# Plonky3/Plonky3-recursion

Hardware: AMD Instinct MI355X
Metric: prove_next_layer ms + Poseidon2 perms/s, KoalaBear 2^20-row circuit, 1/8 GPU (lower is better)
Workload: dtype u32 Montgomery (31-bit prime field, degree-4 extension); Poseidon2 hashing as exact integers in f64; 1 GPU; prove_next_layer (verifier-circuit run on the device + prove_all_tables) of the synthetic koala-bear 2^20-row recursion layer: tables const/public/alu/poseidon2/recompose, FRI blowup 4, arity<=4, 54 queries, 15-bit PoW; circuit inputs + NextLayerPrepCache resident in HBM; field=koala-bear, log_height=20, independent_proofs=1, proof_bytes=612900, parallelism=1 independent proofs, one per GPU, no data-path collective

## Files before the change

__graft_entry__.py:

```python
import os
import subprocess
import sys

ROOT = os.path.dirname(os.path.abspath(__file__))
CSRC = os.path.join(ROOT, "plonky3_recursion_amd", "csrc")
LIB = os.path.join(ROOT, "plonky3_recursion_amd", "libp3r_hip.so")
KNOBS_LIB = os.path.join(ROOT, "plonky3_recursion_amd", "knobs", "libp3r_hip.so")
HIP_SOURCES = ["p3r_core.hip", "tu_lde.hip", "tu_quotient.hip", "tu_logup.hip", "tu_mmcs4.hip", "prep_device.hip"]


def _stale(target, deps):
    if not os.path.exists(target):
        return True
    t = os.path.getmtime(target)
    return any(os.path.getmtime(d) > t for d in deps)


def _deps_of(obj):
    dep = obj + ".d"
    if not os.path.exists(dep):
        return None
    txt = open(dep).read().replace("\\\n", " ")
    return [p for p in txt.split(":", 1)[1].split() if p]


def build():
    hipcc = os.environ.get("HIPCC", "/opt/rocm/bin/hipcc")
    flags = ["-O3", "-std=c++17", "--offload-arch=gfx950", "-fPIC", "-pthread"]
    objdir = os.path.join(CSRC, ".build")
    os.makedirs(objdir, exist_ok=True)
    os.makedirs(os.path.dirname(KNOBS_LIB), exist_ok=True)
    shared = ["prep_device.hip", "tu_quotient.hip", "tu_logup.hip", "tu_mmcs4.hip"]
    knobbed = ["p3r_core.hip", "tu_lde.hip"]
    units = [(src, src + ".o", []) for src in HIP_SOURCES]
    units += [(src, src.replace(".hip", ".knobs.o"), ["-DP3R_TUNING_KNOBS"]) for src in knobbed]
    test_only = ["tu_prims_test.hip", "tu_p2f_test.hip"]
    units += [(src, src.replace(".hip", ".knobs.o"), ["-DP3R_TUNING_KNOBS"]) for src in test_only]
    pending = []
    for src, objname, extra in units:
        obj = os.path.join(objdir, objname)
        deps = _deps_of(obj)
        if deps is None or not all(os.path.exists(d) for d in deps) or _stale(obj, deps):
            pending.append((obj, [hipcc] + flags + extra + ["-MD", "-MF", obj + ".d", "-c", "-o", obj, os.path.join(CSRC, src)]))
    running, failed = [], None
    max_jobs = max(1, min(len(pending), (os.cpu_count() or 2)))
    while pending or running:
        while pending and len(running) < max_jobs:
            obj, cmd = pending.pop(0)
            running.append((obj, subprocess.Popen(cmd, cwd=CSRC)))
        obj, proc = running.pop(0)
        if proc.wait() != 0:
            for p in (obj, obj + ".d"):
                if os.path.exists(p):
                    os.remove(p)
            failed = failed or subprocess.CalledProcessError(proc.returncode, proc.args)
    if failed:
        raise failed
    for lib, objs in ((LIB, [s + ".o" for s in HIP_SOURCES]),
                      (KNOBS_LIB, [s.replace(".hip", ".knobs.o") for s in knobbed + test_only] + [s + ".o" for s in shared])):
        paths = [os.path.join(objdir, o) for o in objs]
        if _stale(lib, paths):
            subprocess.run([hipcc] + flags + ["-shared", "-o", lib] + paths, check=True, cwd=CSRC)
    subprocess.run(["make", "-C", os.path.join(ROOT, "oracle")], check=True,
                   stdout=subprocess.DEVNULL)
    subprocess.run(["make", "-C", os.path.join(ROOT, "harness")], check=True,
                   stdout=subprocess.DEVNULL, stderr=subprocess.DEVNULL)
    subprocess.run(["make", "-C", os.path.join(ROOT, "examples")], check=True, stdout=subprocess.DEVNULL)
    chk = os.path.join(ROOT, "tools", "microbench", "zk_fill_check")
    srcs = [chk + ".hip", os.path.join(CSRC, "kernels_zk.hip.h"), os.path.join(CSRC, "zk_rand.h")]
    if not os.path.exists(chk) or any(os.path.getmtime(f) > os.path.getmtime(chk) for f in srcs):
        subprocess.run([hipcc, "--offload-arch=gfx950", "-O3", "-std=c++17", "-w", "-I", CSRC, "-o", chk, chk + ".hip"], check=True)
    if ROOT not in sys.path:
        sys.path.insert(0, ROOT)
    import plonky3_recursion_amd
    from plonky3_recursion_amd import _lib
    _lib.load()


def smoke():
    if ROOT not in sys.path:
        sys.path.insert(0, ROOT)
    sys.path.insert(0, os.path.join(ROOT, "tests"))
    import numpy as np
    import oracle_lib
    import plonky3_recursion_amd as p3r

    field = "koala-bear"
    ctx = p3r.Context(field=field)
    orc = oracle_lib.Oracle()
    rng = np.random.default_rng(0)
    n = 256
    p = oracle_lib.MODULUS[field]
    inputs = rng.integers(0, p, size=(n, 16), dtype=np.uint32)
    new_start = (rng.random(n) < 0.2).astype(np.uint8)
    merkle = (rng.random(n) < 0.7).astype(np.uint8)
    bit = rng.integers(0, 2, size=n, dtype=np.uint8)
    idx = rng.integers(0, p, size=n, dtype=np.uint32)
    g = oracle_lib.GENERATOR[field]
    tr = ctx.generate_trace_rows_device(inputs, new_start, merkle, bit, idx)
    lde = ctx.coset_lde_batch_device(tr, 2, g)
    cap, tree = ctx.commit_device([lde])
    o_tr = orc.trace_rows(field, inputs, new_start, merkle, bit, idx)
    assert np.array_equal(tr.download(), o_tr), "trace fill mismatch"
    o_lde = orc.coset_lde(field, o_tr, 2, g)
    assert np.array_equal(lde.download(), o_lde), "LDE mismatch"
    ocap, otree = orc.commit(field, [o_lde], 0)
    assert np.array_equal(cap, ocap), "MMCS commitment mismatch"
    opened, proof = tree.open_batch(321)
    assert orc.verify(field, cap, [o_lde.shape], 321, opened, proof), "opening rejected by oracle"
    tree.free()
    ctx.close()
    print("smoke ok: trace fill + LDE + MMCS commit/open bit-exact vs oracle")

    import circuit_lib
    import harness_lib
    import layer_lib
    import harness_adapters as wl
    fri = dict(log_blowup=2, max_log_arity=2, cap_height=0, log_final_poly_len=2, commit_pow_bits=0,
               query_pow_bits=6, num_queries=8)
# ... 30 lines not shown
```

plonky3_recursion_amd/csrc/context.h:

```cpp
#pragma once
#include <hip/hip_runtime.h>

#include <algorithm>
#include <array>
#include <atomic>
#include <cstdarg>
#include <cstdio>
#include <cstring>
#include <exception>
#include <functional>
#include <map>
#include <memory>
#include <chrono>
#include <mutex>
#include <stdexcept>
#include <string>
#include <thread>
#include <tuple>
#include <vector>

#include "../../include/p3r.h"
#include "field.h"
#include "poseidon2.h"
#include "proof_layout.h"
// ... 356 lines not shown
};

struct DevBuf {
  uint32_t* p = nullptr;
  size_t n = 0;
  std::shared_ptr<DevPool> pool;
  DevBuf() = default;
  explicit DevBuf(size_t cells) { alloc(cells); }
  DevBuf(const DevBuf&) = delete;
  DevBuf& operator=(const DevBuf&) = delete;
  DevBuf(DevBuf&& o) noexcept : p(o.p), n(o.n), pool(std::move(o.pool)) { o.p = nullptr; o.n = 0; }
  DevBuf& operator=(DevBuf&& o) noexcept {
    if (this != &o) { release(); p = o.p; n = o.n; pool = std::move(o.pool); o.p = nullptr; o.n = 0; }
    return *this;
  }
  ~DevBuf() { release(); }
  void alloc(size_t cells) {
    release();
    if (cells) {
      pool = tls_pool();
      if (!pool) fail(P3R_EINVAL, "device allocation outside a p3r API call");
      p = static_cast<uint32_t*>(pool->get(cells * sizeof(uint32_t)));
    }
    n = cells;
  }
  void release() {
    if (p) pool->put(p, n * sizeof(uint32_t));
    p = nullptr;
    n = 0;
    pool.reset();
  }
};

inline int log2_exact(size_t x, const char* what) {
  if (x == 0 || (x & (x - 1))) fail(P3R_EINVAL, "%s (%zu) must be a power of two", what, x);
  int l = 0;
  while ((size_t(1) << l) < x) ++l;
  return l;
}

}

struct p3r_dmat {
  p3r::DevBuf buf;
  uint32_t* d = nullptr;
  size_t h = 0, w = 0;
};

struct p3r_p2_dev {
  size_t n = 0;
  std::unique_ptr<p3r_dmat> inputs;
  p3r::DevBuf flags;
  p3r::DevBuf seed;
};

struct p3r_tree {
  std::vector<const p3r_dmat*> mats;
  std::vector<std::unique_ptr<p3r_dmat>> owned;
  int salt_elems = 0;
  std::vector<std::unique_ptr<p3r_dmat>> salt_owned;
  p3r::DevBuf phase_salts;
  size_t phase_salt_stride = 0, phase_rows = 0;
  int log_max_h = 0;
  int cap_height = 0;
  size_t total_width = 0;
  std::vector<p3r::DevBuf> layers;
  int arity = 2;
  std::vector<p3r::MmcsLevel> levels;
  std::vector<size_t> layer_n;
};

namespace p3r {
struct ProfRec {
  const char* name;
  hipEvent_t a, b;
};
}

struct p3r_ctx {
  p3r_config cfg{};
  std::shared_ptr<p3r::DevPool> pool = std::make_shared<p3r::DevPool>();
  bool prof_enabled = false;
  std::vector<p3r::ProfRec> prof;
  std::vector<std::pair<std::string, double>> stage_ms;
  std::string cur_stage;
  double cur_stage_t0 = 0;
  int partial_rounds = 0;
  hipStream_t stream = nullptr;
  int n_cus = 256;
  p3r::DevBuf rc;
  p3r::DevBuf rc_f64;
  const double* rcd() const { return reinterpret_cast<const double*>(rc_f64.p); }
  size_t rcd_w32_at = 0;
  const double* rcd_w32() const { return rcd() + rcd_w32_at; }
  p3r::DevBuf p2_diag;
  std::vector<uint32_t> rc_canonical;
  std::vector<uint8_t> fri_log_arities;
  p3r::ProofLayout proof_layout;
  std::vector<uint32_t> rc_mont_host;
  std::string err;
  bool w32_diag_builtin = false;
  bool w32_unacknowledged = false;
  uint64_t zk_nonce = 0;
  uint32_t zk_key[8] = {0, 0, 0, 0, 0, 0, 0, 0};
  std::vector<uint8_t> pending_proof;
  p3r::HostStage stage;
  p3r::HostLanding landing;
  p3r::HostPost post;
  std::map<std::string, p3r::DevBuf> const_tables;

  std::map<std::pair<int, int>, p3r::DevBuf> tw_sub;
  std::map<std::pair<int, int>, std::pair<p3r::DevBuf, p3r::DevBuf>> tw4;
  std::map<std::tuple<int, int, uint32_t>, std::pair<p3r::DevBuf, p3r::DevBuf>> pre;
};

inline hipError_t fetch_small(p3r_ctx* ctx, const uint32_t* src, size_t words, uint32_t* dst) {
  if (words == 0) return hipSuccess;
  if (words <= p3r::HostPost::kWords) {
    const uint32_t* got = nullptr;
    p3r::host_mark("fetch: posted, waiting for the GPU");
    hipError_t e = ctx->post.post(ctx->stream, src, words, &got);
    p3r::host_mark("fetch: arrived");
    if (e != hipSuccess) return e;
    std::memcpy(dst, got, words * 4);
    return hipSuccess;
  }
  return p3r::copy_sync(ctx->stream, dst, src, words * 4, hipMemcpyDeviceToHost);
}
```

plonky3_recursion_amd/csrc/kernels_fri_reduce.hip.h:

```cpp
#pragma once
#include "kernels_stark.hip.h"

namespace p3r {

template <int DC>
struct FriInvJobT {
  uint32_t* inv;
  uint64_t h;
  int log_h;
  uint32_t w_h;
  uint32_t w_4;
  EW<DC> z;
  uint32_t block0;
};
using FriInvJob = FriInvJobT<4>;
template <class PP, int DC = 4>
__global__ void __launch_bounds__(kBlock)
k_fri_inv_points(const FriInvJobT<DC>* __restrict__ jobs, int n_jobs, uint32_t gen) {
  using F = Fp<PP>;
  using E = typename Chal<PP, DC>::type;
  const int j = find_job(jobs, n_jobs);
  const FriInvJobT<DC>& job = jobs[j];
  const size_t h = job.h, r0 = ((size_t)(blockIdx.x - job.block0) * kBlock + threadIdx.x) * 4;
  if (r0 >= h) return;
  const E z = e4_load<PP, DC>(job.z);
  E x[4], v[4];
  const F x0 = F::raw(gen) * F::raw(job.w_h).pow(bit_reverse((uint32_t)r0, job.log_h));
  const F x2 = x0 * F::raw(job.w_4);
  x[0] = z - E::from_base(x0);
  x[1] = z + E::from_base(x0);
  x[2] = z - E::from_base(x2);
  x[3] = z + E::from_base(x2);
  inv4<PP>(x, v);
  const gptr<uint32_t> inv = as_global(job.inv);
#pragma unroll
  for (int m = 0; m < 4; ++m)
    if (r0 + m < h)
#pragma unroll
      for (int k = 0; k < DC; ++k) inv[(size_t)k * h + r0 + m] = v[m].c[k].v;
}

struct FriVsumJob {
  const uint32_t* vals;
  uint32_t* out;
  int w;
};
template <class PP, int DC = 4>
__global__ void __launch_bounds__(kBlock)
k_fri_vsum(const FriVsumJob* __restrict__ jobs, const uint32_t* __restrict__ apow_tab ) {
  using F = Fp<PP>;
  using E = typename Chal<PP, DC>::type;
  __shared__ uint32_t sh[kBlock / 64][DC];
  const FriVsumJob job = jobs[blockIdx.x];
  const gptr<const uint32_t> vals = as_global(job.vals);
  E acc = E::zero();
  for (int c = threadIdx.x; c < job.w; c += kBlock) {
    E ap, v;
#pragma unroll
    for (int k = 0; k < DC; ++k) {
      ap.c[k] = F::raw(apow_tab[DC * c + k]);
      v.c[k] = F::raw(vals[DC * c + k]);
    }
    acc += ap * v;
  }
  const int lane = threadIdx.x & 63, wave = threadIdx.x >> 6;
#pragma unroll
  for (int k = 0; k < DC; ++k) {
    F x = acc.c[k];
#pragma unroll
    for (int off = 32; off > 0; off >>= 1) x += F::raw(__shfl_down(x.v, off));
    if (lane == 0) sh[wave][k] = x.v;
  }
  __syncthreads();
  if (threadIdx.x < DC) {
    F x = F::zero();
#pragma unroll
    for (int wv = 0; wv < kBlock / 64; ++wv) x += F::raw(sh[wv][threadIdx.x]);
    as_global(job.out)[threadIdx.x] = x.v;
  }
}

template <int DC>
struct FriReduceMatT {
  const uint32_t* mat;
  int w, n_points;
  const uint32_t* inv[2];
  const uint32_t* v[2];
  EW<DC> off[2];
};
using FriReduceMat = FriReduceMatT<4>;
struct FriReduceJob {
  uint32_t* ro;
  uint64_t h;
  uint32_t mat0, n_mats;
  uint32_t block0;
};
template <class PP, int DC = 4>
__global__ void __launch_bounds__(kBlock)
k_fri_reduce_pre(const FriReduceJob* __restrict__ jobs, int n_jobs, const FriReduceMatT<DC>* __restrict__ mats,
                 const uint32_t* __restrict__ apow_tab ) {
  using F = Fp<PP>;
  using E = typename Chal<PP, DC>::type;
  const int j = find_job(jobs, n_jobs);
  const FriReduceJob job = jobs[j];
  const size_t h = job.h, r = (size_t)(blockIdx.x - job.block0) * kBlock + threadIdx.x;
  if (r >= h) return;
  auto apow = [&](int c) {
    E ap;
#pragma unroll
    for (int k = 0; k < DC; ++k) ap.c[k] = F::raw(apow_tab[DC * c + k]);
    return ap;
  };
  E acc = E::zero();
  for (uint32_t m = 0; m < job.n_mats; ++m) {
    const FriReduceMatT<DC>& a = mats[job.mat0 + m];
    const gptr<const uint32_t> mat = as_global(a.mat);
    const int w = a.w;
    E S = E::zero(), S2 = E::zero();
    int c = 0;
    for (; c + 3 < w; c += 4) {
      const F m0 = F::raw(mat[(size_t)c * h + r]), m1 = F::raw(mat[(size_t)(c + 1) * h + r]);
      const F m2 = F::raw(mat[(size_t)(c + 2) * h + r]), m3 = F::raw(mat[(size_t)(c + 3) * h + r]);
      S += E::dot2_base(apow(c), m0, apow(c + 1), m1);
      S2 += E::dot2_base(apow(c + 2), m2, apow(c + 3), m3);
    }
    for (; c + 1 < w; c += 2)
      S += E::dot2_base(apow(c), F::raw(mat[(size_t)c * h + r]), apow(c + 1), F::raw(mat[(size_t)(c + 1) * h + r]));
    if (c < w) S += apow(c) * F::raw(mat[(size_t)c * h + r]);
    S += S2;
    for (int p = 0; p < a.n_points; ++p) {
      E inv;
#pragma unroll
      for (int k = 0; k < DC; ++k) inv.c[k] = F::raw(as_global(a.inv[p])[(size_t)k * h + r]);
      E V;
#pragma unroll
      for (int k = 0; k < DC; ++k) V.c[k] = F::raw(as_global(a.v[p])[k]);
      acc += e4_load<PP, DC>(a.off[p]) * (V - S) * inv;
    }
  }
#pragma unroll
  for (int k = 0; k < DC; ++k) as_global(job.ro)[(size_t)k * h + r] = acc.c[k].v;
}

}
```

plonky3_recursion_amd/csrc/profile.h:

```cpp
#pragma once
#include <chrono>

#include "context.h"

namespace p3r {

inline void prof_clear(p3r_ctx* ctx) {
  for (auto& r : ctx->prof) {
    (void)hipEventDestroy(r.a);
    (void)hipEventDestroy(r.b);
  }
  ctx->prof.clear();
  ctx->stage_ms.clear();
  ctx->cur_stage.clear();
}

inline void prof_stage(p3r_ctx* ctx, const char* name) {
  p3r::host_mark(name ? name : "stage end");
  if (!ctx->prof_enabled) return;
  (void)hipStreamSynchronize(ctx->stream);
  const double now = std::chrono::duration<double, std::milli>(std::chrono::steady_clock::now().time_since_epoch()).count();
  if (!ctx->cur_stage.empty()) {
    bool found = false;
    for (auto& kv : ctx->stage_ms)
      if (kv.first == ctx->cur_stage) { kv.second += now - ctx->cur_stage_t0; found = true; }
    if (!found) ctx->stage_ms.emplace_back(ctx->cur_stage, now - ctx->cur_stage_t0);
  }
  ctx->cur_stage = name ? name : "";
  ctx->cur_stage_t0 = now;
}

inline void prof_count(p3r_ctx* ctx, const char* name, double v) {
  if (!ctx->prof_enabled) return;
  const std::string key = std::string("count:") + name;
  for (auto& kv : ctx->stage_ms)
    if (kv.first == key) { kv.second += v; return; }
  ctx->stage_ms.emplace_back(key, v);
}

struct ProfScope {
  p3r_ctx* ctx;
  hipEvent_t a = nullptr, b = nullptr;
  const char* name;
  ProfScope(p3r_ctx* c, const char* n) : ctx(c), name(n) {
    if (!ctx->prof_enabled) return;
    if (hipEventCreate(&a) != hipSuccess || hipEventCreate(&b) != hipSuccess) {
      a = b = nullptr;
      return;
    }
    (void)hipEventRecord(a, ctx->stream);
  }
  ~ProfScope() {
    if (!a) return;
    (void)hipEventRecord(b, ctx->stream);
    ctx->prof.push_back(ProfRec{name, a, b});
  }
};

}
```

plonky3_recursion_amd/csrc/prove_impl.hip.h:

```cpp
#include "host_transcript.h"
#include "kernels_stark.hip.h"
#include "kernels_fri_reduce.hip.h"
#include "kernels_zk.hip.h"
#include "open_impl.hip.h"

struct p3r_prep {
  std::vector<p3r::AirParams> airs;
  std::vector<std::unique_ptr<p3r_dmat>> traces;
  std::vector<std::unique_ptr<p3r_dmat>> evals;
  std::vector<std::unique_ptr<p3r_dmat>> ldes;
  std::vector<size_t> heights;
  int zk_codewords = -1;
  const p3r_dmat* committed(size_t i) const { return evals.empty() ? traces[i].get() : evals[i].get(); }
  std::unique_ptr<p3r_tree> tree;
  std::vector<uint32_t> cap_canonical;
};

namespace {

template <class PP, int DC = 4>
EW<DC> to_e4(const typename Chal<PP, DC>::type& e) { return e4_store<PP, DC>(e); }

template <class PP, int DC = 4>
std::vector<typename Chal<PP, DC>::type> download_ef(p3r_ctx* ctx, const uint32_t* dev, size_t count) {
  std::vector<uint32_t> raw(count * DC);
  P3R_HIP(fetch_small(ctx, dev, raw.size(), raw.data()));
  std::vector<typename Chal<PP, DC>::type> out(count);
  for (size_t i = 0; i < count; ++i)
    for (int k = 0; k < DC; ++k) out[i].c[k] = Fp<PP>::raw(raw[i * DC + k]);
  return out;
}

inline ZkKey zk_key_of(const p3r_ctx* ctx, uint64_t nonce) {
  ZkKey k{};
  for (int i = 0; i < 8; ++i) k.k[i] = ctx->zk_key[i];
  k.nonce_lo = (uint32_t)nonce; k.nonce_hi = (uint32_t)(nonce >> 32);
  return k;
}

template <class PP>
void launch_zk_tiles(p3r_ctx* ctx, std::vector<ZkTileJob>& jobs, const ZkKey& key, const char* family) {
  uint64_t blocks = 0;
  for (auto& j : jobs) {
    if (2 * (uint64_t)(j.w2 | 1u) > kZkTileWords) fail(P3R_EUNSUPPORTED, "ZK fill of a matrix of %u columns", j.w2);
    j.log_tr = zk_tile_log_rows(j.rows, j.w2);
    j.block0 = (uint32_t)blocks;
    blocks += j.rows >> j.log_tr;
  }
  if (blocks >= (uint64_t(1) << 31)) fail(P3R_EUNSUPPORTED, "ZK fill launch of %llu tiles", (unsigned long long)blocks);
  if (!blocks) return;
  DevBuf d_jobs((jobs.size() * sizeof(ZkTileJob) + 3) / 4);
  P3R_HIP(ctx->stage.upload(ctx->stream, d_jobs.p, jobs.data(), jobs.size() * sizeof(ZkTileJob)));
  ProfScope ps(ctx, family);
  hipLaunchKernelGGL(k_zk_fill_tiles<PP>, dim3((unsigned)blocks), dim3(kBlock), 0, ctx->stream, reinterpret_cast<const ZkTileJob*>(d_jobs.p),
                     (int)jobs.size(), key);
  P3R_HIP(hipGetLastError());
}

template <class PP>
std::vector<std::unique_ptr<p3r_dmat>> draw_salts(p3r_ctx* ctx, const std::vector<const p3r_dmat*>& mats, int salt_round, const ZkKey& key) {
  const uint32_t S = ctx->cfg.mmcs_salt_elems;
  std::vector<std::unique_ptr<p3r_dmat>> out;
  std::vector<ZkTileJob> tj;
  for (size_t i = 0; i < mats.size(); ++i) {
    out.push_back(dmat_alloc(mats[i]->h, S));
    ZkTileJob j{};
    j.dst = out.back()->d; j.rows = mats[i]->h; j.w2 = S; j.mode = 1; j.stride = 1;
    j.stream = zk_stream_id(salt_round, i);
    tj.push_back(j);
  }
  launch_zk_tiles<PP>(ctx, tj, key, "mmcs_salts");
  return out;
}

template <class PP>
std::unique_ptr<p3r_tree> commit_dmats(p3r_ctx* ctx, const std::vector<const p3r_dmat*>& mats,
                                       std::vector<uint32_t>& cap_mont, int salt_round = -1, const ZkKey* key = nullptr) {
  auto tree = std::make_unique<p3r_tree>();
  tree->mats = mats;
  if (ctx->cfg.mmcs_salt_elems) {
    if (salt_round < 0 || !key) fail(P3R_EHIP, "internal: a commit without its salt stream under a hiding MMCS");
    tree->salt_elems = (int)ctx->cfg.mmcs_salt_elems;
    tree->salt_owned = draw_salts<PP>(ctx, mats, salt_round, *key);
    tree->mats.clear();
    for (size_t i = 0; i < mats.size(); ++i) { tree->mats.push_back(mats[i]); tree->mats.push_back(tree->salt_owned[i].get()); }
// ... 501 lines not shown
        m.z = {zeta};
        if (r == &prep_round || r == &perm_round || (r == &main_round && air_uses_next(prep->airs[m.inst])))
          m.z.push_back(zeta * F::two_adic_generator(log_n[m.inst]));
        m.job = op.open(m.ev->d, m.ev->h, (int)m.ev->w, m.shift, m.z);
      }
    auto all = op.finish();
    launch_inv_points();
    for (Round* r : rounds())
      for (Mat& m : r->mats)
        for (auto& pv : all[m.job]) {
          for (auto& v : pv) ch.observe_ext(v);
          m.vals.emplace_back(pv.begin(), pv.end() - R);
          m.codewords.emplace_back(pv.end() - R, pv.end());
        }
    check_at_zeta();
  }

  static std::array<uint64_t, 6> inv_key(int lh, const E& z) {
    std::array<uint64_t, 6> key{(uint64_t)lh, 0, 0, 0, 0, 0};
    for (int k = 0; k < DC; ++k) key[1 + k] = z.c[k].v;
    return key;
  }

  void launch_inv_points() {
    std::vector<FriInvJobT<DC>> inv_jobs;
    uint32_t inv_blocks = 0;
    for (Round* r : rounds())
      for (const Mat& m : r->mats) {
        const int lh = log_e[m.inst] + log_blowup;
        for (const E& z : m.z) {
          const auto key = inv_key(lh, z);
          if (inv_cache.count(key)) continue;
          inv_keep.emplace_back((size_t)DC << lh);
          FriInvJobT<DC> j{};
          j.inv = inv_keep.back().p;
          j.h = uint64_t(1) << lh;
          j.log_h = lh;
          if (lh < 2) fail(P3R_EINVAL, "FRI: an LDE of fewer than four rows");
          j.w_h = F::two_adic_generator(lh).v;
          j.w_4 = F::two_adic_generator(2).v;
          j.z = to_e4<PP, DC>(z);
          j.block0 = inv_blocks;
          inv_blocks += blocks_for((size_t(1) << lh) / 4);
          inv_jobs.push_back(j);
          inv_cache.emplace(key, j.inv);
        }
      }
    inv_keep.emplace_back((inv_jobs.size() * sizeof(FriInvJobT<DC>) + 3) / 4);
    P3R_HIP(ctx->stage.upload(ctx->stream, inv_keep.back().p, inv_jobs.data(), inv_jobs.size() * sizeof(FriInvJobT<DC>)));
    ProfScope ps(ctx, "fri_inv_points");
    hipLaunchKernelGGL((k_fri_inv_points<PP, DC>), dim3(inv_blocks), dim3(kBlock), 0, ctx->stream,
                       reinterpret_cast<const FriInvJobT<DC>*>(inv_keep.back().p), (int)inv_jobs.size(), gen.v);
    P3R_HIP(hipGetLastError());
  }

  void check_at_zeta() {
    E l_beta_pow[kMaxExtD + 1];
    for (int j = 0; j <= kMaxExtD; ++j) l_beta_pow[j] = e4_load<PP, DC>(lc.beta_pow[j]);
    const E l_prefix = e4_load<PP, DC>(lc.prefix);
    std::vector<std::vector<std::vector<E>>> inst_chunks(ni);
    for (const Mat& m : quot_round.mats) inst_chunks[m.inst].push_back(m.vals[0]);
    static const std::vector<E> empty;
    for (size_t i = 0; i < ni; ++i) {
      const auto& omain = main_round.mats[i].vals;
      const Mat* pm = perm_mat(i);
      ZetaInstance<PP, DC> zi{&omain[0], omain.size() > 1 ? &omain[1] : nullptr, &prep_round.mats[i].vals[0],
                          &prep_round.mats[i].vals[1], pm ? &pm->vals[0] : &empty, pm ? &pm->vals[1] : &empty,
                          &inst_chunks[i], pm ? &terminals[i] : nullptr};
      try {
        check_instance_at_zeta<PP, DC>(prep->airs[i], layouts[i], log_n[i], zi, alpha, zeta, l_prefix, l_beta_pow,
                                   ctx->rc_mont_host.data(), i, zk);
      } catch (const VerifyFailure& e) {
        fail(P3R_EINVAL, "the traces do not satisfy the constraints (%s)", e.what());
      }
    }
    E tsum = E::zero();
    for (const Mat& m : perm_round.mats) tsum += terminals[m.inst];
    if (!tsum.is_zero()) fail(P3R_EINVAL, "the traces do not satisfy the constraints (global lookup sum is not zero)");
  }

  void fri_reduce() {
    prof_stage(ctx, "fri_reduce");
    const E fri_alpha = ch.sample_ext();
    size_t max_w = 1, n_opened = 0;
    for (Round* r : rounds())
      for (const Mat& m : r->mats) { max_w = std::max(max_w, m.lde->w); ++n_opened; }
    std::vector<E> fa_pow(max_w + 1);
    fa_pow[0] = E::one();
    for (size_t c = 1; c <= max_w; ++c) fa_pow[c] = fa_pow[c - 1] * fri_alpha;
    d_fapow.alloc(max_w * DC);
    {
      std::vector<uint32_t> h(max_w * DC);
      for (size_t c = 0; c < max_w; ++c)
        for (int k = 0; k < DC; ++k) h[c * DC + k] = fa_pow[c].c[k].v;
      P3R_HIP(ctx->stage.upload(ctx->stream, d_fapow.p, h.data(), h.size() * 4));
    }
    std::map<int, std::vector<FriReduceMatT<DC>>> by_height;
    std::vector<DevBuf> keep;
    std::vector<FriVsumJob> vsum_jobs;
    DevBuf vsums(2 * DC * n_opened);
    for (Round* r : rounds())
      for (const Mat& m : r->mats) {
        const int lh = log_e[m.inst] + log_blowup;
        auto f = ros.find(lh);
        if (f == ros.end()) f = ros.emplace(lh, std::make_pair(E::one(), DevBuf((size_t)DC << lh))).first;
        FriReduceMatT<DC> a{};
        a.mat = m.lde->d;
        a.w = (int)m.lde->w;
        a.n_points = (int)m.z.size();
        E ap = f->second.first;
        for (size_t p = 0; p < m.z.size(); ++p) {
          a.inv[p] = inv_cache.at(inv_key(lh, m.z[p]));
          a.v[p] = vsums.p + DC * vsum_jobs.size();
          vsum_jobs.push_back({op.values_dev(m.job, (int)p), vsums.p + DC * vsum_jobs.size(), (int)m.ev->w});
          a.off[p] = to_e4<PP, DC>(ap);
          ap *= fa_pow[m.lde->w];
        }
        f->second.first = ap;
        by_height[lh].push_back(a);
      }
    std::vector<FriReduceMatT<DC>> mats;
    std::vector<FriReduceJob> jobs;
    uint32_t blocks = 0;
    for (auto& kv : by_height) {
      FriReduceJob j{};
      j.ro = ros[kv.first].second.p;
      j.h = uint64_t(1) << kv.first;
      j.mat0 = (uint32_t)mats.size();
      j.n_mats = (uint32_t)kv.second.size();
      j.block0 = blocks;
      blocks += blocks_for(size_t(1) << kv.first);
      jobs.push_back(j);
      mats.insert(mats.end(), kv.second.begin(), kv.second.end());
    }
    const size_t b_mats = mats.size() * sizeof(FriReduceMatT<DC>), b_jobs = jobs.size() * sizeof(FriReduceJob),
                 b_vsum = vsum_jobs.size() * sizeof(FriVsumJob);
    const size_t o_jobs = (b_mats + 15) & ~size_t(15), o_vsum = (o_jobs + b_jobs + 15) & ~size_t(15);
    std::vector<unsigned char> blob(o_vsum + b_vsum);
    std::memcpy(blob.data(), mats.data(), b_mats);
    std::memcpy(blob.data() + o_jobs, jobs.data(), b_jobs);
    std::memcpy(blob.data() + o_vsum, vsum_jobs.data(), b_vsum);
    keep.emplace_back((blob.size() + 3) / 4);
    unsigned char* d_blob = reinterpret_cast<unsigned char*>(keep.back().p);
    P3R_HIP(ctx->stage.upload(ctx->stream, d_blob, blob.data(), blob.size()));
    const auto* d_mats = reinterpret_cast<const FriReduceMatT<DC>*>(d_blob);
    const auto* d_jobs = reinterpret_cast<const FriReduceJob*>(d_blob + o_jobs);
    const auto* d_vsum = reinterpret_cast<const FriVsumJob*>(d_blob + o_vsum);
    {
      ProfScope ps(ctx, "fri_reduce");
      hipLaunchKernelGGL((k_fri_vsum<PP, DC>), dim3((unsigned)vsum_jobs.size()), dim3(kBlock), 0, ctx->stream, d_vsum,
                         d_fapow.p);
      hipLaunchKernelGGL((k_fri_reduce_pre<PP, DC>), dim3(blocks), dim3(kBlock), 0, ctx->stream, d_jobs, (int)jobs.size(),
                         d_mats, d_fapow.p);
    }
    P3R_HIP(hipGetLastError());
  }

  void fri_commit_phase() {
    prof_stage(ctx, "fri_commit_phase");
    std::vector<int> heights;
    for (auto& kv : ros) heights.push_back(kv.first);
    std::sort(heights.rbegin(), heights.rend());
    log_max = heights[0];
    const int log_final = (int)cfg.log_final_poly_len + log_blowup;
    folded = std::move(ros[log_max].second);
    size_t next_h = 1;
    int log_cur = log_max;
    const bool device_transcript = cfg.cap_height == 0 && cfg.commit_pow_bits == 0 && ch.in_buf.empty();
    d_tstate.alloc(P2_WIDTH);
    d_phase.alloc((DC + P2_DIGEST) * kMaxPhases);
    uint32_t* const d_betas = d_phase.p;
    uint32_t* const d_caps = d_phase.p + DC * kMaxPhases;
    if (device_transcript) {
      uint32_t st[P2_WIDTH];
      for (int k = 0; k < P2_WIDTH; ++k) st[k] = ch.state[k].v;
      P3R_HIP(ctx->stage.upload(ctx->stream, d_tstate.p, st, sizeof st));
    }
    while (log_cur > log_final) {
      int log_next = next_h < heights.size() ? heights[next_h] : -1;
      int la = fri_log_arity(ctx->fri_log_arities, phases.size(), (int)cfg.max_log_arity, log_cur, log_final, log_next);
      if (la < 0) fail(P3R_EINVAL, "fri_log_arities does not fit the proof: phase %zu at height 2^%d", phases.size(), log_cur);
      if (la > 4) fail(P3R_EUNSUPPORTED, "max_log_arity > 4 is not supported");
      const size_t arity = size_t(1) << la, rows = (size_t(1) << log_cur) >> la;
      Phase ph{la, rows};
      commit_phase_leaves(ph, log_cur);
      const size_t pi = phases.size();
      if (pi >= kMaxPhases) fail(P3R_EUNSUPPORTED, "more than %zu FRI commit phases", kMaxPhases);
      TranscriptStep step{d_tstate.p, d_betas + DC * pi, d_caps + P2_DIGEST * pi};
      step.dc = DC;
      mmcs_build_levels<PP>(ctx, ph.tree.get(), nullptr, device_transcript ? &step : nullptr);
      if (device_transcript) {
        if (!step.done)
          hipLaunchKernelGGL(k_fri_transcript_step<PP>, dim3(1), dim3(64), 0, ctx->stream, ph.tree->layers.back().p,
                             step.state, step.beta, step.cap, ctx->rc.p, ctx->p2_diag.p, DC);
      } else {
        ph.cap = mmcs_cap_mont(ctx, ph.tree.get());
        for (uint32_t v : ph.cap) ch.observe(F::raw(v));
        commit_pow_witnesses.push_back(grind_witness<PP>(ctx, ch, (int)cfg.commit_pow_bits));
        const E beta = ch.sample_ext();
        uint32_t bw[DC];
        for (int k = 0; k < DC; ++k) bw[k] = beta.c[k].v;
        P3R_HIP(ctx->stage.upload(ctx->stream, d_betas + DC * pi, bw, sizeof bw));
      }
      DevBuf out(DC * rows);
      FriFoldArgs fa{};
      fa.in = folded.p; fa.out = out.p; fa.rows = rows; fa.log_rows = log_cur - la;
      fa.beta = d_betas + DC * pi;
      const bool roll = next_h < heights.size() && heights[next_h] == log_cur - la;
      fa.roll = roll ? ros[heights[next_h]].second.p : nullptr;
      fa.w_inv = F::two_adic_generator(log_cur).inv().v;
      const F omega = F::two_adic_generator(la);
      for (int s = 0; s < la; ++s) {
        F om_s = omega.pow(uint64_t(1) << s);
        for (int j = 0; j < (int)(arity >> (s + 1)); ++j)
          fa.tw_inv[s][j] = om_s.pow(bit_reverse(2 * j, la - s)).inv().v;
      }
      fa.neg_half = (-(F::from_canonical(2).inv())).v;
      {
        ProfScope ps(ctx, "fri_fold");
        static constexpr void (*kFold[4])(FriFoldArgs) = {k_fri_fold<PP, DC, 1>, k_fri_fold<PP, DC, 2>, k_fri_fold<PP, DC, 3>,
                                                          k_fri_fold<PP, DC, 4>};
        hipLaunchKernelGGL(kFold[la - 1], dim3(blocks_for(rows)), dim3(kBlock), 0, ctx->stream, fa);
      }
      P3R_HIP(hipGetLastError());
      if (roll) ++next_h;
      ph.folded_in = std::move(folded);
      folded = std::move(out);
      log_cur -= la;
      phases.push_back(std::move(ph));
    }
    if (next_h != heights.size()) fail(P3R_EINVAL, "FRI: an input height was never rolled in");
    final_polynomial(log_cur, device_transcript);
    for (auto& c : final_poly) ch.observe_ext(c);
    for (auto& ph : phases) ch.observe(F::from_canonical((uint32_t)ph.la));
    query_pow_witness = grind_witness<PP>(ctx, ch, (int)cfg.query_pow_bits);
  }

  void commit_phase_leaves(Phase& ph, int log_cur) {
// ... 299 lines not shown
```

Baseline: 25.83 ms.

## Compute FRI reduced openings on trace-height matrices then LDE the combination

For unit-shift (trace-domain) matrices, the alpha-weighted column combination is now computed at trace height, and only the combined 1-2 extension columns are LDE'd to full height. This replaces reading every wide LDE column at blowup height. A post kernel subtracts the LDE'd combination and weighted opened-value sums, then multiplies by the inverse denominators. The old path remains for zk/salted configs or under a tuning knob. The cost is extra kernel launches and a small coset LDE of the combined columns.

```diff
diff --git a/__graft_entry__.py b/__graft_entry__.py
--- a/__graft_entry__.py
+++ b/__graft_entry__.py
@@ -34,7 +34,7 @@
     knobbed = ["p3r_core.hip", "tu_lde.hip"]
     units = [(src, src + ".o", []) for src in HIP_SOURCES]
     units += [(src, src.replace(".hip", ".knobs.o"), ["-DP3R_TUNING_KNOBS"]) for src in knobbed]
-    test_only = ["tu_prims_test.hip", "tu_p2f_test.hip"]
+    test_only = ["tu_prims_test.hip", "tu_p2f_test.hip", "tu_fri_reduce_test.hip"]
     units += [(src, src.replace(".hip", ".knobs.o"), ["-DP3R_TUNING_KNOBS"]) for src in test_only]
     pending = []
     for src, objname, extra in units:
diff --git a/plonky3_recursion_amd/csrc/context.h b/plonky3_recursion_amd/csrc/context.h
--- a/plonky3_recursion_amd/csrc/context.h
+++ b/plonky3_recursion_amd/csrc/context.h
@@ -462,6 +462,7 @@
   std::shared_ptr<p3r::DevPool> pool = std::make_shared<p3r::DevPool>();
   bool prof_enabled = false;
   std::vector<p3r::ProfRec> prof;
+  const char* prof_family = nullptr;
   std::vector<std::pair<std::string, double>> stage_ms;
   std::string cur_stage;
   double cur_stage_t0 = 0;
diff --git a/plonky3_recursion_amd/csrc/fri_reduce_impl.hip.h b/plonky3_recursion_amd/csrc/fri_reduce_impl.hip.h
--- /dev/null
+++ b/plonky3_recursion_amd/csrc/fri_reduce_impl.hip.h
@@ -0,0 +1,226 @@
+#pragma once
+#include <cstring>
+#include <map>
+
+#include "kernels_fri_reduce.hip.h"
+#include "profile.h"
+#include "tu_api.h"
+
+namespace p3r {
+namespace {
+
+inline unsigned fri_blocks(size_t n) { return (unsigned)((n + kBlock - 1) / kBlock); }
+
+struct FriOpenedMat {
+  const p3r_dmat* ev;
+  const p3r_dmat* lde;
+  bool unit_shift;
+  int n_points;
+  const uint32_t* inv[2];
+  const uint32_t* vals[2];
+};
+
+struct ProfFamily {
+  p3r_ctx* ctx;
+  ProfFamily(p3r_ctx* c, const char* name) : ctx(c) { ctx->prof_family = name; }
+  ~ProfFamily() { ctx->prof_family = nullptr; }
+};
+
+template <class PP, int DC>
+void fri_reduced_openings(p3r_ctx* ctx, const std::vector<FriOpenedMat>& opened, const typename Chal<PP, DC>::type& fri_alpha,
+                          bool trace_side, DevBuf& d_fapow, std::map<int, std::pair<typename Chal<PP, DC>::type, DevBuf>>& ros) {
+  using F = Fp<PP>;
+  using E = typename Chal<PP, DC>::type;
+  size_t max_w = 1;
+  for (const FriOpenedMat& m : opened) max_w = std::max(max_w, m.lde->w);
+  std::vector<E> fa_pow(max_w + 1);
+  fa_pow[0] = E::one();
+  for (size_t c = 1; c <= max_w; ++c) fa_pow[c] = fa_pow[c - 1] * fri_alpha;
+  d_fapow.alloc(max_w * DC);
+  {
+    std::vector<uint32_t> h(max_w * DC);
+    for (size_t c = 0; c < max_w; ++c)
+      for (int k = 0; k < DC; ++k) h[c * DC + k] = fa_pow[c].c[k].v;
+    P3R_HIP(ctx->stage.upload(ctx->stream, d_fapow.p, h.data(), h.size() * 4));
+  }
+  std::vector<FriVsumJob> vsum_jobs;
+  DevBuf vsums(2 * DC * std::max<size_t>(opened.size(), 1));
+  struct Term { const FriOpenedMat* m; EW<DC> off[2]; const uint32_t* v[2]; };
+  std::map<int, std::vector<Term>> by_height;
+  for (const FriOpenedMat& m : opened) {
+    const int lh = log2_exact(m.lde->h, "LDE height");
+    auto f = ros.find(lh);
+    if (f == ros.end()) f = ros.emplace(lh, std::make_pair(E::one(), DevBuf((size_t)DC << lh))).first;
+    Term t{&m, {}, {}};
+    E ap = f->second.first;
+    for (int p = 0; p < m.n_points; ++p) {
+      t.v[p] = vsums.p + DC * vsum_jobs.size();
+      vsum_jobs.push_back({m.vals[p], vsums.p + DC * vsum_jobs.size(), (int)m.ev->w});
+      t.off[p] = e4_store<PP, DC>(ap);
+      ap *= fa_pow[m.lde->w];
+    }
+    f->second.first = ap;
+    by_height[lh].push_back(t);
+  }
+  if (vsum_jobs.empty()) return;
+  std::vector<DevBuf> keep;
+  struct Blob {
+    std::vector<unsigned char> bytes;
+    size_t add(const void* p, size_t n) {
+      const size_t at = (bytes.size() + 15) & ~size_t(15);
+      bytes.resize(at + n);
+      if (n) std::memcpy(bytes.data() + at, p, n);
+      return at;
+    }
+  } blob;
+  auto upload_blob = [&]() -> const unsigned char* {
+    keep.emplace_back((blob.bytes.size() + 3) / 4);
+    P3R_HIP(ctx->stage.upload(ctx->stream, keep.back().p, blob.bytes.data(), blob.bytes.size()));
+    return reinterpret_cast<const unsigned char*>(keep.back().p);
+  };
+  if (!trace_side) {
+    std::vector<FriReduceMatT<DC>> mats;
+    std::vector<FriReduceJob> jobs;
+    uint32_t blocks = 0;
+    for (auto& kv : by_height) {
+      FriReduceJob j{};
+      j.ro = ros[kv.first].second.p;
+      j.h = uint64_t(1) << kv.first;
+      j.mat0 = (uint32_t)mats.size();
+      j.n_mats = (uint32_t)kv.second.size();
+      j.block0 = blocks;
+      blocks += fri_blocks(size_t(1) << kv.first);
+      jobs.push_back(j);
+      for (const Term& t : kv.second) {
+        FriReduceMatT<DC> a{};
+        a.mat = t.m->lde->d;
+        a.w = (int)t.m->lde->w;
+        a.n_points = t.m->n_points;
+        for (int p = 0; p < a.n_points; ++p) { a.inv[p] = t.m->inv[p]; a.v[p] = t.v[p]; a.off[p] = t.off[p]; }
+        mats.push_back(a);
+      }
+    }
+    const size_t o_mats = blob.add(mats.data(), mats.size() * sizeof(FriReduceMatT<DC>));
+    const size_t o_jobs = blob.add(jobs.data(), jobs.size() * sizeof(FriReduceJob));
+    const size_t o_vsum = blob.add(vsum_jobs.data(), vsum_jobs.size() * sizeof(FriVsumJob));
+    const unsigned char* d_blob = upload_blob();
+    ProfScope ps(ctx, "fri_reduce");
+    hipLaunchKernelGGL((k_fri_vsum<PP, DC>), dim3((unsigned)vsum_jobs.size()), dim3(kBlock), 0, ctx->stream,
+                       reinterpret_cast<const FriVsumJob*>(d_blob + o_vsum), d_fapow.p);
+    hipLaunchKernelGGL((k_fri_reduce_pre<PP, DC>), dim3(blocks), dim3(kBlock), 0, ctx->stream,
+                       reinterpret_cast<const FriReduceJob*>(d_blob + o_jobs), (int)jobs.size(),
+                       reinterpret_cast<const FriReduceMatT<DC>*>(d_blob + o_mats), d_fapow.p);
+    P3R_HIP(hipGetLastError());
+    return;
+  }
+
+  std::vector<FriCombineMatT<DC>> cmats, dmats;
+  std::vector<FriCombineJob> cjobs;
+  std::vector<FriPostJob> pjobs;
+  std::vector<FriWsumTermT<DC>> wterms;
+  std::vector<FriWsumJob> wjobs;
+  std::vector<std::unique_ptr<p3r_dmat>> ts;
+  std::vector<size_t> t_job;
+  std::vector<int> t_bits;
+  DevBuf wsums(2 * DC * by_height.size());
+  uint32_t cblocks = 0, pblocks = 0;
+  for (auto& kv : by_height) {
+    const size_t h = size_t(1) << kv.first;
+    FriPostJob pj{};
+    pj.ro = ros[kv.first].second.p;
+    pj.h = h;
+    pj.mat0 = (uint32_t)dmats.size();
+    FriCombineJob cj{};
+    cj.mat0 = (uint32_t)cmats.size();
+    std::vector<FriWsumTermT<DC>> wt[2];
+    for (const Term& t : kv.second) {
+      FriCombineMatT<DC> a{};
+      a.w = (int)t.m->lde->w;
+      a.n_points = t.m->n_points;
+      for (int p = 0; p < a.n_points; ++p) {
+        int s = 0;
+        while (s < pj.n_slots && pj.inv[s] != t.m->inv[p]) ++s;
+        if (s == 2) fail(P3R_EUNSUPPORTED, "FRI: more than two opening points at one height");
+        if (s == pj.n_slots) pj.inv[pj.n_slots++] = t.m->inv[p];
+        a.slot[p] = s;
+        a.off[p] = t.off[p];
+        wt[s].push_back({t.v[p], t.off[p]});
+      }
+      if (t.m->unit_shift) {
+        if (t.m->ev->w != t.m->lde->w || t.m->ev->h > h) fail(P3R_EHIP, "internal: an opened matrix and its LDE disagree");
+        if (cj.n_mats && t.m->ev->h != cj.h) fail(P3R_EUNSUPPORTED, "FRI: trace heights %zu and %zu extend to one LDE height", (size_t)cj.h, t.m->ev->h);
+        cj.h = t.m->ev->h;
+        a.mat = t.m->ev->d;
+        cmats.push_back(a);
+        ++cj.n_mats;
+      } else {
+        a.mat = t.m->lde->d;
+        dmats.push_back(a);
+        ++pj.n_mats;
+      }
+    }
+    for (int s = 0; s < pj.n_slots; ++s) {
+      pj.w[s] = wsums.p + DC * wjobs.size();
+      wjobs.push_back({wsums.p + DC * wjobs.size(), (uint32_t)wterms.size(), (uint32_t)wt[s].size()});
+      wterms.insert(wterms.end(), wt[s].begin(), wt[s].end());
+    }
+    if (cj.n_mats) {
+      ts.push_back(dmat_alloc(cj.h, (size_t)pj.n_slots * DC));
+      cj.t = ts.back()->d;
+      cj.n_slots = pj.n_slots;
+      cj.block0 = cblocks;
+      cblocks += fri_blocks(cj.h);
+      cjobs.push_back(cj);
+      t_job.push_back(pjobs.size());
+      t_bits.push_back(kv.first - log2_exact(cj.h, "trace height"));
+    }
+    pj.block0 = pblocks;
+    pblocks += fri_blocks(h);
+    pjobs.push_back(pj);
+  }
+  ProfFamily family(ctx, "fri_reduce");
+  const size_t o_vsum = blob.add(vsum_jobs.data(), vsum_jobs.size() * sizeof(FriVsumJob));
+  const size_t o_wterms = blob.add(wterms.data(), wterms.size() * sizeof(FriWsumTermT<DC>));
+  const size_t o_wjobs = blob.add(wjobs.data(), wjobs.size() * sizeof(FriWsumJob));
+  const size_t o_cmats = blob.add(cmats.data(), cmats.size() * sizeof(FriCombineMatT<DC>));
+  const size_t o_cjobs = blob.add(cjobs.data(), cjobs.size() * sizeof(FriCombineJob));
+  const size_t o_dmats = blob.add(dmats.data(), dmats.size() * sizeof(FriCombineMatT<DC>));
+  const unsigned char* d_blob = upload_blob();
+  {
+    ProfScope ps(ctx, "fri_reduce");
+    hipLaunchKernelGGL((k_fri_vsum<PP, DC>), dim3((unsigned)vsum_jobs.size()), dim3(kBlock), 0, ctx->stream,
+                       reinterpret_cast<const FriVsumJob*>(d_blob + o_vsum), d_fapow.p);
+    hipLaunchKernelGGL((k_fri_wsum<PP, DC>), dim3((unsigned)wjobs.size()), dim3(64), 0, ctx->stream,
+                       reinterpret_cast<const FriWsumJob*>(d_blob + o_wjobs), reinterpret_cast<const FriWsumTermT<DC>*>(d_blob + o_wterms));
+    if (cblocks)
+      hipLaunchKernelGGL((k_fri_combine<PP, DC>), dim3(cblocks), dim3(kBlock), 0, ctx->stream,
+                         reinterpret_cast<const FriCombineJob*>(d_blob + o_cjobs), (int)cjobs.size(),
+                         reinterpret_cast<const FriCombineMatT<DC>*>(d_blob + o_cmats), d_fapow.p);
+    P3R_HIP(hipGetLastError());
+  }
+  std::vector<std::unique_ptr<p3r_dmat>> t_ldes(ts.size());
+  for (size_t i = 0; i < ts.size(); ++i) {
+    if (t_ldes[i]) continue;
+    std::vector<LdeItem> items;
+    std::vector<size_t> which;
+    for (size_t k = i; k < ts.size(); ++k)
+      if (!t_ldes[k] && t_bits[k] == t_bits[i]) { items.push_back({ts[k].get(), PP::GEN}); which.push_back(k); }
+    auto out = coset_lde_batch<PP>(ctx, items, t_bits[i]);
+    for (size_t k = 0; k < which.size(); ++k) {
+      t_ldes[which[k]] = std::move(out[k]);
+      pjobs[t_job[which[k]]].t = t_ldes[which[k]]->d;
+    }
+  }
+  keep.emplace_back((pjobs.size() * sizeof(FriPostJob) + 3) / 4);
+  P3R_HIP(ctx->stage.upload(ctx->stream, keep.back().p, pjobs.data(), pjobs.size() * sizeof(FriPostJob)));
+  {
+    ProfScope ps(ctx, "fri_reduce");
+    hipLaunchKernelGGL((k_fri_reduce_post<PP, DC>), dim3(pblocks), dim3(kBlock), 0, ctx->stream,
+                       reinterpret_cast<const FriPostJob*>(keep.back().p), (int)pjobs.size(),
+                       reinterpret_cast<const FriCombineMatT<DC>*>(d_blob + o_dmats), d_fapow.p);
+    P3R_HIP(hipGetLastError());
+  }
+}
+
+}
+}
diff --git a/plonky3_recursion_amd/csrc/kernels_fri_reduce.hip.h b/plonky3_recursion_amd/csrc/kernels_fri_reduce.hip.h
--- a/plonky3_recursion_amd/csrc/kernels_fri_reduce.hip.h
+++ b/plonky3_recursion_amd/csrc/kernels_fri_reduce.hip.h
@@ -80,6 +80,32 @@
   }
 }
 
+template <class PP, int DC>
+__device__ __forceinline__ typename Chal<PP, DC>::type fri_row_sum(gptr<const uint32_t> mat, int w, size_t h, size_t r,
+                                                                   const uint32_t* __restrict__ apow_tab) {
+  using F = Fp<PP>;
+  using E = typename Chal<PP, DC>::type;
+  auto apow = [&](int c) {
+    E ap;
+#pragma unroll
+    for (int k = 0; k < DC; ++k) ap.c[k] = F::raw(apow_tab[DC * c + k]);
+    return ap;
+  };
+  E S = E::zero(), S2 = E::zero();
+  int c = 0;
+  for (; c + 3 < w; c += 4) {
+    const F m0 = F::raw(mat[(size_t)c * h + r]), m1 = F::raw(mat[(size_t)(c + 1) * h + r]);
+    const F m2 = F::raw(mat[(size_t)(c + 2) * h + r]), m3 = F::raw(mat[(size_t)(c + 3) * h + r]);
+    S += E::dot2_base(apow(c), m0, apow(c + 1), m1);
+    S2 += E::dot2_base(apow(c + 2), m2, apow(c + 3), m3);
+  }
+  for (; c + 1 < w; c += 2)
+    S += E::dot2_base(apow(c), F::raw(mat[(size_t)c * h + r]), apow(c + 1), F::raw(mat[(size_t)(c + 1) * h + r]));
+  if (c < w) S += apow(c) * F::raw(mat[(size_t)c * h + r]);
+  S += S2;
+  return S;
+}
+
 template <int DC>
 struct FriReduceMatT {
   const uint32_t* mat;
@@ -105,29 +131,12 @@
   const FriReduceJob job = jobs[j];
   const size_t h = job.h, r = (size_t)(blockIdx.x - job.block0) * kBlock + threadIdx.x;
   if (r >= h) return;
-  auto apow = [&](int c) {
-    E ap;
-#pragma unroll
-    for (int k = 0; k < DC; ++k) ap.c[k] = F::raw(apow_tab[DC * c + k]);
-    return ap;
-  };
   E acc = E::zero();
   for (uint32_t m = 0; m < job.n_mats; ++m) {
     const FriReduceMatT<DC>& a = mats[job.mat0 + m];
     const gptr<const uint32_t> mat = as_global(a.mat);
     const int w = a.w;
-    E S = E::zero(), S2 = E::zero();
-    int c = 0;
-    for (; c + 3 < w; c += 4) {
-      const F m0 = F::raw(mat[(size_t)c * h + r]), m1 = F::raw(mat[(size_t)(c + 1) * h + r]);
-      const F m2 = F::raw(mat[(size_t)(c + 2) * h + r]), m3 = F::raw(mat[(size_t)(c + 3) * h + r]);
-      S += E::dot2_base(apow(c), m0, apow(c + 1), m1);
-      S2 += E::dot2_base(apow(c + 2), m2, apow(c + 3), m3);
-    }
-    for (; c + 1 < w; c += 2)
-      S += E::dot2_base(apow(c), F::raw(mat[(size_t)c * h + r]), apow(c + 1), F::raw(mat[(size_t)(c + 1) * h + r]));
-    if (c < w) S += apow(c) * F::raw(mat[(size_t)c * h + r]);
-    S += S2;
+    const E S = fri_row_sum<PP, DC>(mat, w, h, r, apow_tab);
     for (int p = 0; p < a.n_points; ++p) {
       E inv;
 #pragma unroll
@@ -142,4 +151,132 @@
   for (int k = 0; k < DC; ++k) as_global(job.ro)[(size_t)k * h + r] = acc.c[k].v;
 }
 
-}
+template <int DC>
+struct FriCombineMatT {
+  const uint32_t* mat;
+  int w, n_points;
+  int slot[2];
+  EW<DC> off[2];
+};
+struct FriCombineJob {
+  uint32_t* t;
+  uint64_t h;
+  uint32_t mat0, n_mats;
+  int n_slots;
+  uint32_t block0;
+};
+template <class PP, int DC = 4>
+__global__ void __launch_bounds__(kBlock)
+k_fri_combine(const FriCombineJob* __restrict__ jobs, int n_jobs, const FriCombineMatT<DC>* __restrict__ mats,
+              const uint32_t* __restrict__ apow_tab ) {
+  using E = typename Chal<PP, DC>::type;
+  const int j = find_job(jobs, n_jobs);
+  const FriCombineJob job = jobs[j];
+  const size_t h = job.h, r = (size_t)(blockIdx.x - job.block0) * kBlock + threadIdx.x;
+  if (r >= h) return;
+  E T0 = E::zero(), T1 = E::zero();
+  for (uint32_t m = 0; m < job.n_mats; ++m) {
+    const FriCombineMatT<DC>& a = mats[job.mat0 + m];
+    const E S = fri_row_sum<PP, DC>(as_global(a.mat), a.w, h, r, apow_tab);
+    for (int p = 0; p < a.n_points; ++p) {
+      const E x = e4_load<PP, DC>(a.off[p]) * S;
+      if (a.slot[p] == 0) T0 += x;
+      else T1 += x;
+    }
+  }
+  const gptr<uint32_t> t = as_global(job.t);
+#pragma unroll
+  for (int k = 0; k < DC; ++k) t[(size_t)k * h + r] = T0.c[k].v;
+  if (job.n_slots > 1)
+#pragma unroll
+    for (int k = 0; k < DC; ++k) t[(size_t)(DC + k) * h + r] = T1.c[k].v;
+}
+
+template <int DC>
+struct FriWsumTermT {
+  const uint32_t* v;
+  EW<DC> off;
+};
+struct FriWsumJob {
+  uint32_t* out;
+  uint32_t term0, n_terms;
+};
+template <class PP, int DC = 4>
+__global__ void __launch_bounds__(64)
+k_fri_wsum(const FriWsumJob* __restrict__ jobs, const FriWsumTermT<DC>* __restrict__ terms) {
+  using F = Fp<PP>;
+  using E = typename Chal<PP, DC>::type;
+  const FriWsumJob job = jobs[blockIdx.x];
+  E acc = E::zero();
+  for (uint32_t i = threadIdx.x; i < job.n_terms; i += 64) {
+    const FriWsumTermT<DC>& t = terms[job.term0 + i];
+    E v;
+#pragma unroll
+    for (int k = 0; k < DC; ++k) v.c[k] = F::raw(as_global(t.v)[k]);
+    acc += e4_load<PP, DC>(t.off) * v;
+  }
+#pragma unroll
+  for (int k = 0; k < DC; ++k) {
+    F x = acc.c[k];
+#pragma unroll
+    for (int off = 32; off > 0; off >>= 1) x += F::raw(__shfl_down(x.v, off));
+    if (threadIdx.x == 0) as_global(job.out)[k] = x.v;
+  }
+}
+
+struct FriPostJob {
+  uint32_t* ro;
+  const uint32_t* t;
+  uint64_t h;
+  int n_slots;
+  const uint32_t* inv[2];
+  const uint32_t* w[2];
+  uint32_t mat0, n_mats;
+  uint32_t block0;
+};
+template <class PP, int DC = 4>
+__global__ void __launch_bounds__(kBlock)
+k_fri_reduce_post(const FriPostJob* __restrict__ jobs, int n_jobs, const FriCombineMatT<DC>* __restrict__ mats,
+                  const uint32_t* __restrict__ apow_tab ) {
+  using F = Fp<PP>;
+  using E = typename Chal<PP, DC>::type;
+  const int j = find_job(jobs, n_jobs);
+  const FriPostJob job = jobs[j];
+  const size_t h = job.h, r = (size_t)(blockIdx.x - job.block0) * kBlock + threadIdx.x;
+  if (r >= h) return;
+  E A[2] = {E::zero(), E::zero()};
+#pragma unroll
+  for (int s = 0; s < 2; ++s)
+    if (s < job.n_slots) {
+#pragma unroll
+      for (int k = 0; k < DC; ++k) A[s].c[k] = F::raw(as_global(job.w[s])[k]);
+      if (job.t) {
+        E t;
+#pragma unroll
+        for (int k = 0; k < DC; ++k) t.c[k] = F::raw(as_global(job.t)[(size_t)(s * DC + k) * h + r]);
+        A[s] -= t;
+      }
+    }
+  for (uint32_t m = 0; m < job.n_mats; ++m) {
+    const FriCombineMatT<DC>& a = mats[job.mat0 + m];
+    const E S = fri_row_sum<PP, DC>(as_global(a.mat), a.w, h, r, apow_tab);
+    for (int p = 0; p < a.n_points; ++p) {
+      const E x = e4_load<PP, DC>(a.off[p]) * S;
+      if (a.slot[p] == 0) A[0] -= x;
+      else A[1] -= x;
+    }
+  }
+  E acc = E::zero();
+#pragma unroll
+  for (int s = 0; s < 2; ++s)
+    if (s < job.n_slots) {
+      E inv;
+#pragma unroll
+      for (int k = 0; k < DC; ++k) inv.c[k] = F::raw(as_global(job.inv[s])[(size_t)k * h + r]);
+      acc += A[s] * inv;
+    }
+#pragma unroll
+  for (int k = 0; k < DC; ++k) as_global(job.ro)[(size_t)k * h + r] = acc.c[k].v;
+}
+
+}
diff --git a/plonky3_recursion_amd/csrc/profile.h b/plonky3_recursion_amd/csrc/profile.h
--- a/plonky3_recursion_amd/csrc/profile.h
+++ b/plonky3_recursion_amd/csrc/profile.h
@@ -42,7 +42,7 @@
   p3r_ctx* ctx;
   hipEvent_t a = nullptr, b = nullptr;
   const char* name;
-  ProfScope(p3r_ctx* c, const char* n) : ctx(c), name(n) {
+  ProfScope(p3r_ctx* c, const char* n) : ctx(c), name(c->prof_family ? c->prof_family : n) {
     if (!ctx->prof_enabled) return;
     if (hipEventCreate(&a) != hipSuccess || hipEventCreate(&b) != hipSuccess) {
       a = b = nullptr;
diff --git a/plonky3_recursion_amd/csrc/prove_impl.hip.h b/plonky3_recursion_amd/csrc/prove_impl.hip.h
--- a/plonky3_recursion_amd/csrc/prove_impl.hip.h
+++ b/plonky3_recursion_amd/csrc/prove_impl.hip.h
@@ -1,6 +1,6 @@
 #include "host_transcript.h"
 #include "kernels_stark.hip.h"
-#include "kernels_fri_reduce.hip.h"
+#include "fri_reduce_impl.hip.h"
 #include "kernels_zk.hip.h"
 #include "open_impl.hip.h"
 
@@ -668,78 +668,20 @@
   void fri_reduce() {
     prof_stage(ctx, "fri_reduce");
     const E fri_alpha = ch.sample_ext();
-    size_t max_w = 1, n_opened = 0;
-    for (Round* r : rounds())
-      for (const Mat& m : r->mats) { max_w = std::max(max_w, m.lde->w); ++n_opened; }
-    std::vector<E> fa_pow(max_w + 1);
-    fa_pow[0] = E::one();
-    for (size_t c = 1; c <= max_w; ++c) fa_pow[c] = fa_pow[c - 1] * fri_alpha;
-    d_fapow.alloc(max_w * DC);
-    {
-      std::vector<uint32_t> h(max_w * DC);
-      for (size_t c = 0; c < max_w; ++c)
-        for (int k = 0; k < DC; ++k) h[c * DC + k] = fa_pow[c].c[k].v;
-      P3R_HIP(ctx->stage.upload(ctx->stream, d_fapow.p, h.data(), h.size() * 4));
-    }
-    std::map<int, std::vector<FriReduceMatT<DC>>> by_height;
-    std::vector<DevBuf> keep;
-    std::vector<FriVsumJob> vsum_jobs;
-    DevBuf vsums(2 * DC * n_opened);
+    std::vector<FriOpenedMat> opened;
     for (Round* r : rounds())
       for (const Mat& m : r->mats) {
         const int lh = log_e[m.inst] + log_blowup;
-        auto f = ros.find(lh);
-        if (f == ros.end()) f = ros.emplace(lh, std::make_pair(E::one(), DevBuf((size_t)DC << lh))).first;
-        FriReduceMatT<DC> a{};
-        a.mat = m.lde->d;
-        a.w = (int)m.lde->w;
-        a.n_points = (int)m.z.size();
-        E ap = f->second.first;
+        FriOpenedMat o{m.ev, m.lde, m.shift == F::one(), (int)m.z.size(), {}, {}};
         for (size_t p = 0; p < m.z.size(); ++p) {
-          a.inv[p] = inv_cache.at(inv_key(lh, m.z[p]));
-          a.v[p] = vsums.p + DC * vsum_jobs.size();
-          vsum_jobs.push_back({op.values_dev(m.job, (int)p), vsums.p + DC * vsum_jobs.size(), (int)m.ev->w});
-          a.off[p] = to_e4<PP, DC>(ap);
-          ap *= fa_pow[m.lde->w];
+          o.inv[p] = inv_cache.at(inv_key(lh, m.z[p]));
+          o.vals[p] = op.values_dev(m.job, (int)p);
         }
-        f->second.first = ap;
-        by_height[lh].push_back(a);
-      }
-    std::vector<FriReduceMatT<DC>> mats;
-    std::vector<FriReduceJob> jobs;
-    uint32_t blocks = 0;
-    for (auto& kv : by_height) {
-      FriReduceJob j{};
-      j.ro = ros[kv.first].second.p;
-      j.h = uint64_t(1) << kv.first;
-      j.mat0 = (uint32_t)mats.size();
-      j.n_mats = (uint32_t)kv.second.size();
-      j.block0 = blocks;
-      blocks += blocks_for(size_t(1) << kv.first);
-      jobs.push_back(j);
-      mats.insert(mats.end(), kv.second.begin(), kv.second.end());
-    }
-    const size_t b_mats = mats.size() * sizeof(FriReduceMatT<DC>), b_jobs = jobs.size() * sizeof(FriReduceJob),
-                 b_vsum = vsum_jobs.size() * sizeof(FriVsumJob);
-    const size_t o_jobs = (b_mats + 15) & ~size_t(15), o_vsum = (o_jobs + b_jobs + 15) & ~size_t(15);
-    std::vector<unsigned char> blob(o_vsum + b_vsum);
-    std::memcpy(blob.data(), mats.data(), b_mats);
-    std::memcpy(blob.data() + o_jobs, jobs.data(), b_jobs);
-    std::memcpy(blob.data() + o_vsum, vsum_jobs.data(), b_vsum);
-    keep.emplace_back((blob.size() + 3) / 4);
-    unsigned char* d_blob = reinterpret_cast<unsigned char*>(keep.back().p);
-    P3R_HIP(ctx->stage.upload(ctx->stream, d_blob, blob.data(), blob.size()));
-    const auto* d_mats = reinterpret_cast<const FriReduceMatT<DC>*>(d_blob);
-    const auto* d_jobs = reinterpret_cast<const FriReduceJob*>(d_blob + o_jobs);
-    const auto* d_vsum = reinterpret_cast<const FriVsumJob*>(d_blob + o_vsum);
-    {
-      ProfScope ps(ctx, "fri_reduce");
-      hipLaunchKernelGGL((k_fri_vsum<PP, DC>), dim3((unsigned)vsum_jobs.size()), dim3(kBlock), 0, ctx->stream, d_vsum,
-                         d_fapow.p);
-      hipLaunchKernelGGL((k_fri_reduce_pre<PP, DC>), dim3(blocks), dim3(kBlock), 0, ctx->stream, d_jobs, (int)jobs.size(),
-                         d_mats, d_fapow.p);
-    }
-    P3R_HIP(hipGetLastError());
+        opened.push_back(o);
+      }
+    bool trace_side = !zk && !cfg.mmcs_salt_elems;
+    if (tuning_knob("P3R_FRI_REDUCE_ON_LDE")) trace_side = false;
+    fri_reduced_openings<PP, DC>(ctx, opened, fri_alpha, trace_side, d_fapow, ros);
   }
 
   void fri_commit_phase() {
```

Measured after the change: 26.41 ms. 2.2% more time.
